# CMU-SAFARI/AirLift

Measured on AMD Instinct MI355X. Metric: reads/sec remapped (150 bp PE), higher is better.
Workload: dtype u8/int32 (int8 SW lanes, u64 hashes)

## Files before the change

### airlift_amd/csrc/al_dev_ksw2.h

```cpp
#pragma once

#define DPP_ROW_BCAST7 0x157

typedef short al_s2 __attribute__((ext_vector_type(2)));
typedef unsigned short al_u2 __attribute__((ext_vector_type(2)));
__device__ __forceinline__ al_s2 pk_s(uint32_t v) { return __builtin_bit_cast(al_s2, v); }
__device__ __forceinline__ uint32_t pk_u(al_s2 v) { return __builtin_bit_cast(uint32_t, v); }
__device__ __forceinline__ uint32_t pk_add(uint32_t a, uint32_t b) { return pk_u(pk_s(a) + pk_s(b)); }
__device__ __forceinline__ uint32_t pk_sub(uint32_t a, uint32_t b) { return pk_u(pk_s(a) - pk_s(b)); }
__device__ __forceinline__ uint32_t pk_max(uint32_t a, uint32_t b) { return pk_u(__builtin_elementwise_max(pk_s(a), pk_s(b))); }
__device__ __forceinline__ uint32_t pk_min(uint32_t a, uint32_t b) { return pk_u(__builtin_elementwise_min(pk_s(a), pk_s(b))); }
__device__ __forceinline__ uint32_t pk_sar8(uint32_t a) { return pk_u(pk_s(a) >> (al_s2)(8)); }
__device__ __forceinline__ uint32_t pk_minu1(uint32_t a) { uint32_t d; asm("v_pk_min_u16 %0, %1, 1 op_sel_hi:[1,0]" : "=v"(d) : "v"(a)); return d; }
__device__ __forceinline__ uint32_t pk_subsat(uint32_t a, uint32_t b) { uint32_t d; asm("v_pk_sub_u16 %0, %1, %2 clamp" : "=v"(d) : "v"(a), "v"(b)); return d; }
__device__ __forceinline__ uint32_t pk_dec(uint32_t a) { uint32_t d; asm("v_pk_sub_u16 %0, %1, 1 op_sel_hi:[1,0]" : "=v"(d) : "v"(a)); return d; }
__device__ __forceinline__ uint32_t pk_mask_eq(uint32_t t, uint32_t v) { return pk_dec(pk_minu1(t ^ v)); }
__device__ __forceinline__ uint32_t pk_mask_in(uint32_t t, uint32_t lo, uint32_t width) { return pk_dec(pk_minu1(pk_subsat(pk_sub(t, lo), width))); }
__device__ __forceinline__ uint32_t d_bfi(uint32_t mask, uint32_t if_set, uint32_t if_clear) { return (if_set & mask) | (if_clear & ~mask); }
__device__ __forceinline__ uint32_t pk_splat(int v) { return (uint32_t)(v & 0xffff) * 0x00010001u; }
__device__ __forceinline__ uint32_t pk_splat8(int v) { return (uint32_t)((v & 0xff) << 8) * 0x00010001u; }
__device__ __forceinline__ unsigned long long d_grp_any(unsigned long long b) { b |= b >> 8; b |= b >> 4; b |= b >> 2; b |= b >> 1; return b & 0x0001000100010001ull; }

template <int NP, class LT, int DIR = 2, bool EXIT = false>
__device__ __forceinline__ void d_ksw_pk(LT &L, const uint8_t *__restrict__ selE, const uint8_t *__restrict__ selO, const int gl, GroupWs &ws, int qlen, int tlen, const AlParams &P,
                                         int w, int zdrop, int end_bonus, int flag, EzD &ez, bool do_bt = true, unsigned long long *xcnt = nullptr)
{
	int q = P.q, e = P.e, q2 = P.q2, e2 = P.e2;
	if (q2 + e2 < q + e) { int t = q; q = q2; q2 = t; t = e; e = e2; e2 = t; }
	const int qe = q + e;
	const int sc_mch = P.a, sc_mis = -P.b;
	if (w < 0) w = tlen > qlen ? tlen : qlen;
	const int tlen_ = (tlen + 15) / 16;
	int n_col_ = qlen < tlen ? qlen : tlen;
	n_col_ = ((n_col_ < w + 1 ? n_col_ : w + 1) + 15) / 16 + 1;
	int long_thres = e != e2 ? (q2 - q) / (e - e2) - 1 : 0;
	if (q2 + e2 + long_thres * e2 > q + e + long_thres * e) ++long_thres;
	const int long_diff = long_thres * (e - e2) - (q2 - q) - e2;
	const bool right = DIR == 2 ? (flag & EZ_RIGHT) != 0 : DIR == 1;
	const uint32_t M1 = pk_splat8(-q - e), M2 = pk_splat8(-q2 - e2), QE = pk_splat8(q + e), QE2 = pk_splat8(q2 + e2), QQ = pk_splat8(q), QQ2 = pk_splat8(q2), MCH = pk_splat8(sc_mch);
	const uint32_t TG0 = right ? 0x00000000u : 0x00070007u, TG1 = right ? 0x00010001u : 0x00060006u, TG2 = right ? 0x00020002u : 0x00050005u,
// ... 235 lines not shown
		const int rows_run = r < n_rows ? r + 1 : n_rows, need = exit_row >= 0 ? exit_row + 1 : rows_run;
		bool differs = false;
		if (exit_row >= 0) {
			const int smax = (int)L.ezc[0], smax_t = (int)L.ezc[1], smax_q = (int)L.ezc[2], smqe = (int)L.ezc[3], smqe_t = (int)L.ezc[4];
			const bool reach_f = !ez.zdropped && ez.mqe + end_bonus > ez.max, reach_s = smqe + end_bonus > smax;
			differs = smax != ez.max || smax_t != ez.max_t || smax_q != ez.max_q || reach_s != reach_f || (reach_f && smqe_t != ez.mqe_t);
		}
		int wn = need, wr = rows_run;
		const bool full = __ballot(1) == ~0ull;
		if (full) { wn = max(wn, __shfl_xor(wn, 16)); wn = max(wn, __shfl_xor(wn, 32)); wr = max(wr, __shfl_xor(wr, 16)); wr = max(wr, __shfl_xor(wr, 32)); }
		if (gl == 0) {
			const int sv = (int)((long long)(n_rows - need) * 100 / n_rows);
			atomicAdd(xcnt + 0, 1ull); if (differs) atomicAdd(xcnt + 1, 1ull);
			atomicAdd(xcnt + 2, (unsigned long long)n_rows); atomicAdd(xcnt + 3, (unsigned long long)need);
			atomicAdd(xcnt + (sv < 25 ? 6 : 7), (sv < 10 || (sv >= 25 && sv < 40)) ? 1ull : 1ull << 32);
		}
		if (full && threadIdx.x == 0) { atomicAdd(xcnt + 4, (unsigned long long)wr); atomicAdd(xcnt + 5, (unsigned long long)wn); }
	}
	GSYNC();
	if (do_bt) {
		const int rev_cigar = !!(flag & EZ_REV_CIGAR);
		CigW cw{L.ezc, 0, AL_LCIG, ws.ezc, 0xffffffffu};
		if (!ez.zdropped && !(flag & EZ_EXTZ_ONLY)) d_backtrack(ptb, n_col_ * 16, qlen, tlen, w, rev_cigar, tlen - 1, qlen - 1, cw);
		else if (!ez.zdropped && (flag & EZ_EXTZ_ONLY) && ez.mqe + end_bonus > ez.max) { ez.reach_end = 1; d_backtrack(ptb, n_col_ * 16, qlen, tlen, w, rev_cigar, ez.mqe_t, qlen - 1, cw); }
		else if (ez.max_t >= 0 && ez.max_q >= 0) d_backtrack(ptb, n_col_ * 16, qlen, tlen, w, rev_cigar, ez.max_t, ez.max_q, cw);
		ez.n_cigar = cw.n; ws.cur_ezc = cw.c;
	}
	GSYNC();
}
```

### airlift_amd/csrc/al_internal.h

```cpp
#pragma once
#include <stdint.h>
#include <stddef.h>
#include <string>
#include <vector>
#include <memory>
#include <utility>
#include <map>
#include <mutex>
#include "../../include/airlift.h"

#define AL_MAX_K 28
static inline int al_sketch_pos_bits(int k) { const int b = 64 - 2 * k; return b > 22 ? 22 : b; }
static inline bool al_sketch_wide(int k, int max_read_len) { const int pb = al_sketch_pos_bits(k); return k > 25 || max_read_len >= (1 << (pb - 1)); }
#define AL_MAX_READ_LEN 32768
#define AL_SEED_TANDEM    (1ULL<<42)
#define AL_SEED_SEG_SHIFT 48
#define AL_SEED_SEG_MASK  (0xffULL<<AL_SEED_SEG_SHIFT)
#define AL_PARENT_UNSET   (-1)
#define AL_PARENT_TMP_PRI (-2)

struct AlSeq { std::string name; uint64_t offset; uint32_t len; };

struct AlDevIndex {
	uint32_t *S4 = nullptr;
// ... 29 lines not shown
	template <class U, class... A> void construct(U *p, A &&...a) { if constexpr (sizeof...(A) == 0) ::new ((void *)p) U; else ::new ((void *)p) U(std::forward<A>(a)...); }
};
typedef std::vector<char, AlNoInit<char>> AlText;
bool al_fasta_load_parallel(const char *fn, int n_threads, std::vector<AlSeq> &seqs, AlText &ascii);
void al_sketch_host(const uint8_t *codes, uint32_t len, int w, int k, uint32_t rid, std::vector<uint64_t> &hash_out, std::vector<uint64_t> &y_out);

struct AlParams {
	int k, w;
	int seed, bw, max_gap, max_gap_ref, max_frag_len, max_chain_skip, max_chain_iter, min_cnt, min_chain_score;
	float mask_level, pri_ratio, max_clip_ratio;
	int best_n, a, b, q, e, q2, e2, sc_ambi, zdrop, zdrop_inv, end_bonus, min_dp_max;
	int pe_ori, pe_bonus, mid_occ, max_occ;
	int dbg;
	int dbg2;
	int dp_exit;
};

struct AlMatch {
	uint32_t off_lo;
	uint32_t n;
	uint32_t q_pos;
	uint32_t flags;
};

struct AlAnchor { uint64_t x, y; };

#define AL_MAX_CIGAR_INLINE 0

struct AlReg {
	int32_t id, cnt, rid, score;
// ... 43 lines not shown
```

### airlift_amd/csrc/al_kernels_align.hip

```cpp
#include <hip/hip_runtime.h>
#include <string.h>
#include <cstring>
#include <rocprim/rocprim.hpp>
#include <stdio.h>
#include <string.h>
#include <math.h>
#include <vector>
#include <type_traits>
#include "al_internal.h"
#include "al_device.h"
#include "al_runtime.h"
#include "al_dev_regs.h"

#define AL_LREG 6
#define AL_LANC 64
#define AL_LCIG 40
#define AL_LPTB 1280
#define AL_GPB 4
#define GW 16
#define KSW_NEG_INF -0x40000000
#define EZ_RIGHT      0x02
#define EZ_EXTZ_ONLY  0x40
#define EZ_REV_CIGAR  0x80
#define GSYNC() __syncthreads()
// ... 1834 lines not shown
					}
				}
				const int wband = (int)(P.bw * 1.5 + 1.);
				const bool runoff = tl >= ql + wband + 1;
				const bool reach = !runoff && sc + P.end_bonus > mx;
				const int ncig = (reach || pos >= 0) ? 1 : 0;
				ExtOut o; o.max = mx; o.max_q = pos; o.max_t = pos; o.mqe_t = ql - 1;
				o.flags_ncig = (uint32_t)(reach ? 1 : 0) | (uint32_t)(runoff ? 2 : 0) | (uint32_t)ncig << 8; o.cig_off = 0;
				o.cig[0] = ncig ? (uint32_t)(reach ? ql : pos + 1) << 4 : 0; o.cig[1] = o.cig[2] = o.cig[3] = o.cig[4] = o.cig[5] = 0;
				E.outs[jb + side] = o;
				return true;
			};
			if (shortcut(0, jl.qlen, jl.tlen)) jl.pad0 = 1;
			if (shortcut(1, jr.qlen, jr.tlen)) jr.pad0 = 1;
		}
		if (r->cnt > 0 && !((P.dbg >> 18) & 1) && (jl.qlen == 0 || jl.pad0) && (jr.qlen == 0 || jr.pad0)) x.job |= 0x80000000u;
		return 0;
	};
	auto commit = [&](const uint32_t s, const int i, const uint32_t jb, const RegExt &x, const ExtJob &jl, const ExtJob &jr) {
		E.rext[B2 + (uint64_t)s * fw.cap + i] = x;
		E.jobs[jb] = jl; E.jobs[jb + 1] = jr;
		const int c0 = (jl.qlen && !jl.pad0) ? d_job_class(jl.qlen, jl.tlen, lane_ok) : AL_NCLS, c1 = (jr.qlen && !jr.pad0) ? d_job_class(jr.qlen, jr.tlen, lane_ok) : AL_NCLS;
		const uint32_t b0 = (uint32_t)std::min(63, (jl.tlen + 15) / 16), b1 = (uint32_t)std::min(63, (jr.tlen + 15) / 16);
		E.job_key[jb] = c0 < AL_NCLS ? ((uint32_t)c0 << 20 | b0 << 14 | 0u << 13 | (uint32_t)std::min(0x1fff, jl.qlen + jl.tlen)) : 0xffffffffu;
		E.job_key[jb + 1] = c1 < AL_NCLS ? ((uint32_t)c1 << 20 | b1 << 14 | 1u << 13 | (uint32_t)std::min(0x1fff, jr.qlen + jr.tlen)) : 0xffffffffu;
		atomicAdd(&s_hist[c0], 1u); atomicAdd(&s_hist[c1], 1u);
		if (c0 == 7 && b0 <= 16) atomicAdd(&s_sub[b0 <= 12 ? 0 : 1], 1u);
		if (c1 == 7 && b1 <= 16) atomicAdd(&s_sub[b1 <= 12 ? 0 : 1], 1u);
		if (c0 < AL_NCLS) atomicAdd(&s_tl[c0], (unsigned)jl.tlen); if (c1 < AL_NCLS) atomicAdd(&s_tl[c1], (unsigned)jr.tlen);
	};
	auto do_seg = [&](const uint32_t s, const AlReg *regs, const AlAnchor *a) {
		const int qlen = (int)rd_len[r0 + s], n = (int)W.reg_cnt[r0 + s];
		const uint32_t *seq = rd_seq + rd_off[r0 + s];
		if (n > 0 && qlen > qmax) { if (!WAVE || lane == 0) atomicAdd(&G.counters[7], 1ULL << 0); slow = true; return; }
		if (!WAVE) {
			for (int i = 0; i < n; ++i) {
				RegExt x; ExtJob jl, jr; const uint32_t jb = jb0 + 2u * n_done;
				const int code = hit(s, i, regs, a, qlen, seq, jb, x, jl, jr);
				if (code) { if (code == 2) atomicAdd(&G.counters[7], 1ULL << 8); slow = true; return; }
				commit(s, i, jb, x, jl, jr); ++n_done;
// ... 151 lines not shown
		} else {
			const ReadAcc Q{seq, rqlen, job.rev, (int)job.qoff};
			for (int t = gl; t < ql + TMAXJ + 16; t += GW) qr[t] = t < ql ? (uint8_t)Q(ql - 1 - t) : 0;
			for (int i = gl; i < tl; i += GW) L.tbuf[i] = (uint8_t)d_seq4(G.S4, job.toff + (uint64_t)i);
		}
		GSYNC();
		EzD ez; d_ez_reset(ez);
		const int flag = job.kind == 0 ? (EZ_EXTZ_ONLY | EZ_RIGHT | EZ_REV_CIGAR) : EZ_EXTZ_ONLY;
		static_assert(TMAXJ == 16 * NB, "the query pad of JobLds is one block row");
		if constexpr (PK) {
			static_assert(NB % 2 == 0, "two blocks per superblock");
			for (int i = gl; i < ql + 2 * TMAXJ + 16; i += GW) { const uint32_t b0 = L.sq[i]; L.selO[i] = (uint8_t)(b0 < 4 ? 4u + b0 : 0x0du); L.sq[i] = (uint8_t)(b0 < 4 ? b0 : 0x0du); }
			GSYNC();
			const unsigned long long w_act = __ballot(1), w_right = __ballot((flag & EZ_RIGHT) != 0);
			unsigned long long *const xcnt = ((P.dbg2 >> 5) & 1) ? G.counters + 24 : nullptr;
			if (w_right == 0) d_ksw_pk<NB / 2, JobLds<QMAXJ, TMAXJ, PK>, 0, (NB >= 12)>(L, L.sq + TMAXJ, L.selO + TMAXJ, gl, ws, ql, tl, P, bw, P.zdrop, P.end_bonus, flag, ez, true, xcnt);
			else if (w_right == w_act) d_ksw_pk<NB / 2, JobLds<QMAXJ, TMAXJ, PK>, 1, (NB >= 12)>(L, L.sq + TMAXJ, L.selO + TMAXJ, gl, ws, ql, tl, P, bw, P.zdrop, P.end_bonus, flag, ez, true, xcnt);
			else d_ksw_pk<NB / 2, JobLds<QMAXJ, TMAXJ, PK>, 2, (NB >= 12)>(L, L.sq + TMAXJ, L.selO + TMAXJ, gl, ws, ql, tl, P, bw, P.zdrop, P.end_bonus, flag, ez, true, xcnt);
		} else
		d_ksw_reg<NB>(L, gl, ws, ql, tl, P, bw, P.zdrop, P.end_bonus, flag, ez);
		ExtOut o;
		o.max = ez.max; o.max_q = ez.max_q; o.max_t = ez.max_t; o.mqe_t = ez.mqe_t;
		o.flags_ncig = (uint32_t)(ez.reach_end ? 1 : 0) | (uint32_t)(ez.zdropped ? 2 : 0) | (uint32_t)ez.n_cigar << 8; o.cig_off = 0;
		for (int i = 0; i < 6; ++i) o.cig[i] = i < ez.n_cigar ? ws.cur_ezc[i] : 0;
		if (ez.n_cigar > 6) {
			unsigned long long off = 0;
			if (gl == 0) off = atomicAdd(G.arena_cnt, (unsigned long long)ez.n_cigar);
			off = __shfl(off, 0, GW);
			if (off + ez.n_cigar <= G.arena_cap) { for (int i = gl; i < ez.n_cigar; i += GW) G.arena[off + i] = ws.cur_ezc[i]; o.cig_off = (uint32_t)off; }
			else { if (gl == 0) atomicAdd(&G.counters[9], 1ULL); o.cig_off = 0xffffffffu; }
		}
		if (gl == 0) E.outs[j] = o;
		GSYNC();
// ... 975 lines not shown
```

### airlift_amd/csrc/al_runtime.h

```cpp
#pragma once
#include <hip/hip_runtime.h>
#include <stdio.h>
#include <vector>
#include <string>
#include <thread>
#include <chrono>
#include "al_internal.h"

inline bool &al_nomem_flag() { static thread_local bool f = false; return f; }

hipError_t al_dev_malloc(void **p, size_t bytes);
#include <atomic>
std::atomic<size_t> *&al_acct();
struct AlAllocSite { const char *file; int line; };
AlAllocSite &al_alloc_site();
struct AlAllocStat { std::atomic<long long> dev_ns{0}, dev_bytes{0}, dev_calls{0}, host_ns{0}, host_bytes{0}, host_calls{0}; };
AlAllocStat &al_alloc_stat();
void al_dev_free(void *p);
double al_long_batch_cap(double reads);
long long al_dev_reserve_room();
hipError_t al_dev_mem_info(size_t *free_b, size_t *total_b);
int al_dev_guard_check();

template <typename T> struct DevBuf {
// ... 156 lines not shown
```

### airlift_amd/csrc/al_runtime.hip

```cpp
#include <hip/hip_runtime.h>
#include <stdio.h>
#include <stdlib.h>
#include <string.h>
#include <sys/stat.h>
#include <cstring>
#include <rocprim/rocprim.hpp>
#include <algorithm>
#include "al_internal.h"
#include "al_device.h"
#include <mutex>
#include <condition_variable>
#include <thread>
#include <atomic>
#include <map>
#include <vector>
#include "al_runtime.h"
#include "al_dev_sort.h"
#include "al_io.h"

extern "C" __global__ void k_sketch(const uint32_t *, const uint64_t *, const uint32_t *, const uint64_t *, AlAnchor *, uint32_t *, int, int, int, int);
extern "C" __global__ void k_seed(const uint64_t *, int, const uint32_t *, const uint32_t *, const uint64_t *, AlAnchor *, const uint32_t *, AlMatch *, uint32_t *, uint32_t *, int32_t *, const uint32_t *, int, int, int, uint32_t *);
#ifndef AL_SPEC_CAP
#define AL_SPEC_CAP 512
#endif
// ... 378 lines not shown
	for (int i = 0; i < 3; ++i) if (hipStreamCreateWithPriority(&c->aux[i], hipStreamNonBlocking, sp) != hipSuccess || hipEventCreateWithFlags(&c->ev_aux[i], hipEventDisableTiming) != hipSuccess) { delete c; return nullptr; }
	for (int i = 0; i < 3; ++i) if (hipStreamCreateWithFlags(&c->ovl[i], hipStreamNonBlocking) != hipSuccess) { delete c; return nullptr; }
	if (hipStreamCreateWithFlags(&c->spec, hipStreamNonBlocking) != hipSuccess || hipStreamCreateWithFlags(&c->spec2, hipStreamNonBlocking) != hipSuccess) { delete c; return nullptr; }
	for (int i = 0; i < 3; ++i) if (hipEventCreateWithFlags(&c->ev_spec[i], hipEventDisableTiming) != hipSuccess) { delete c; return nullptr; }
	for (int i = 0; i < 5; ++i) if (hipEventCreateWithFlags(&c->ev_ovl[i], hipEventDisableTiming) != hipSuccess) { delete c; return nullptr; }
	if (al_upload_index(mi, device, &c->di) != 0) { delete c; return nullptr; }
	AlParams &P = c->P;
	P.k = mi->k; P.w = mi->w; P.seed = opt->seed; P.bw = opt->bw; P.max_gap = opt->max_gap; P.max_gap_ref = opt->max_gap_ref; P.max_frag_len = opt->max_frag_len;
	P.max_chain_skip = opt->max_chain_skip; P.max_chain_iter = opt->max_chain_iter; P.min_cnt = opt->min_cnt; P.min_chain_score = opt->min_chain_score;
	P.mask_level = opt->mask_level; P.pri_ratio = opt->pri_ratio; P.max_clip_ratio = opt->max_clip_ratio; P.best_n = opt->best_n;
	P.a = opt->a; P.b = opt->b; P.q = opt->q; P.e = opt->e; P.q2 = opt->q2; P.e2 = opt->e2; P.sc_ambi = opt->sc_ambi; P.zdrop = opt->zdrop; P.zdrop_inv = opt->zdrop_inv;
	P.end_bonus = opt->end_bonus; P.min_dp_max = opt->min_dp_max; P.pe_ori = opt->pe_ori; P.pe_bonus = opt->pe_bonus; P.mid_occ = opt->mid_occ; P.max_occ = opt->max_occ;
	{ const char *d = getenv("AL_DBG"); P.dbg = d ? atoi(d) : 0; if (P.dbg) fprintf(stderr, "[airlift] AL_DBG=%d: timing experiment, results are NOT valid\n", P.dbg); }
	{ const char *d = getenv("AL_DBG2"); P.dbg2 = d ? atoi(d) : 0; if (P.dbg2 & ~32) fprintf(stderr, "[airlift] AL_DBG2=%d: timing experiment, results are NOT valid\n", P.dbg2); }
	{ const char *d = getenv("AL_DP_EXIT"); P.dp_exit = d ? atoi(d) != 0 : 1; }
	memset(&c->stat, 0, sizeof(c->stat));
	return c;
}

void al_align_state_free(al_ctx_t *c);
static void ctx_release_buffers(al_ctx_t *c)
{
	if (c->stream) (void)hipStreamSynchronize(c->stream);
	if (c->side) (void)hipStreamSynchronize(c->side);
	for (int i = 0; i < 3; ++i) if (c->aux[i]) (void)hipStreamSynchronize(c->aux[i]);
	for (int i = 0; i < 3; ++i) if (c->ovl[i]) (void)hipStreamSynchronize(c->ovl[i]);
	if (c->spec) (void)hipStreamSynchronize(c->spec);
	if (c->spec2) (void)hipStreamSynchronize(c->spec2);
	(void)hipGetLastError();
	al_align_state_free(c);
// ... 90 lines not shown
	al_parallel_for(c->n_threads, (size_t)n_reads, [&](size_t lo, size_t hi, int) {
		for (size_t i = lo; i < hi; ++i) {
			uint32_t *w = c->h_rd_seq.data() + c->h_rd_off[i]; const char *s = seqs[i]; const int L = qlens[i], nw = (L + 7) / 8 + 1;
			for (int b = 0; b < nw; ++b) {
				uint32_t v = 0; const int j0 = b * 8, j1 = j0 + 8 < L ? j0 + 8 : L;
				if (!c->h_flip[i]) for (int j = j0; j < j1; ++j) v |= (uint32_t)nt4[(unsigned char)s[j]] << ((j & 7) << 2);
				else for (int j = j0; j < j1; ++j) { const unsigned cd = nt4[(unsigned char)s[L - 1 - j]]; v |= (uint32_t)(cd < 4 ? 3 - cd : 4) << ((j & 7) << 2); }
				w[b] = v;
			}
		}
	});
	hipStream_t s = c->stream;
	if (c->rd_seq.ensure(words + 1) || c->rd_off.ensure(n_reads + 1) || c->rd_len.ensure(n_reads + 1) || c->frag_first.ensure(n_frag + 1) || c->frag_hash.ensure(n_frag + 1) ||
	    c->mini_off.ensure(n_reads + 1) || c->mini.ensure(mtot + 1) || c->mini_cnt.ensure(n_reads + 1) || c->match.ensure(mtot + 1) || c->heap_ws.ensure(mtot + 1) ||
	    c->frag_nm.ensure(n_frag + 1) || c->frag_na.ensure(n_frag + 1) || c->frag_rep.ensure(n_frag + 1) || c->frag_nu.ensure(n_frag + 1) || c->a_off.ensure(n_frag + 2) ||
	    c->rechain_list.ensure(n_frag + 1) || c->tmp_u32.ensure(n_frag + 2) || c->tmp_u64.ensure(n_frag + 2) || c->counters.ensure(32)) return -1;
	AL_HIP_CHECK(hipMemcpyAsync(c->rd_seq.p, c->h_rd_seq.data(), (words + 1) * 4, hipMemcpyHostToDevice, s));
	AL_HIP_CHECK(hipMemcpyAsync(c->rd_off.p, c->h_rd_off.data(), (n_reads + 1) * 8, hipMemcpyHostToDevice, s));
	AL_HIP_CHECK(hipMemcpyAsync(c->rd_len.p, c->h_rd_len.data(), (n_reads + 1) * 4, hipMemcpyHostToDevice, s));
	AL_HIP_CHECK(hipMemcpyAsync(c->frag_first.p, c->h_frag_first.data(), (n_frag + 1) * 4, hipMemcpyHostToDevice, s));
	AL_HIP_CHECK(hipMemcpyAsync(c->frag_hash.p, c->h_frag_hash.data(), (n_frag + 1) * 4, hipMemcpyHostToDevice, s));
	AL_HIP_CHECK(hipMemcpyAsync(c->mini_off.p, c->h_mini_off.data(), (n_reads + 1) * 8, hipMemcpyHostToDevice, s));
	AL_HIP_CHECK(hipStreamSynchronize(s));
	return 0;
}

struct CastU64 { __host__ __device__ uint64_t operator()(const uint32_t &v) const { return (uint64_t)v; } };

static int scan_u32_to_u64(al_ctx_t *c, const uint32_t *in, uint64_t *out, int n, hipStream_t st = nullptr, DevBuf<unsigned char> *tmp = nullptr)
{
	hipStream_t s_ = st ? st : c->stream; DevBuf<unsigned char> &T_ = tmp ? *tmp : c->scan_tmp;
// ... 622 lines not shown
				TileSched S; for (int k = 0; k < 6; ++k) { S.ent[k] = 0; S.item[k] = 0; } S.ent[6] = n_tie; S.item[6] = n_tie; S.n_items = n_tie;
				if (chain_tiles(c, c->tie_sorted.p, S, nullptr, lmin, false, lds_ok)) return -1;
			} else if (chain_legacy(c, c->tie_sorted.p, (int)n_tie, lds_ok, nullptr)) return -1;
		}
		if (ev(ST_SEG_MERGE)) return -1;
	}
	AL_HIP_CHECK(hipGetLastError());
	return 0;
}
#undef LCH

int al_run_seed_stages(al_ctx_t *c)
{
	hipStream_t s = c->stream;
	AL_HIP_CHECK(hipSetDevice(c->device));
	AL_HIP_CHECK(hipMemsetAsync(c->counters.p, 0, 32 * sizeof(unsigned long long), s));
	AL_HIP_CHECK(hipEventRecord(c->ev[0], s));
	const int nr = c->n_reads, w = c->mi->w, k = c->mi->k;
	const bool sk_wide = al_sketch_wide(k, c->max_rd_len);
	if (nr > 0) hipLaunchKernelGGL(k_sketch, dim3((nr + 63) / 64), dim3(64), (size_t)w * 64 * (sk_wide ? 12 : 8), s, c->rd_seq.p, c->rd_off.p, c->rd_len.p, c->mini_off.p, c->mini.p, c->mini_cnt.p, nr, w, k, sk_wide ? -1 : al_sketch_pos_bits(k));
	AL_HIP_CHECK(hipEventRecord(c->ev[ST_SKETCH + 1], s));
	if (c->n_frag == 0) { for (int i = ST_SEED; i < ST_N; ++i) AL_HIP_CHECK(hipEventRecord(c->ev[i + 1], s)); return 0; }
	if (c->frag_meta.ensure((size_t)c->n_frag + 1)) return -1;
	hipLaunchKernelGGL(k_frag_meta, dim3((c->n_frag + 255) / 256), dim3(256), 0, s, c->frag_first.p, c->rd_len.p, c->n_frag, c->frag_meta.p);
	if (run_seed_chain(c, nullptr, c->n_frag, c->opt.mid_occ, 0, true)) return -1;
	c->n_rechain = 0;
	if (c->opt.max_occ > c->opt.mid_occ) {
		uint32_t *cnt = (uint32_t *)(c->counters.p + 3);
		hipLaunchKernelGGL(k_rechain_test, dim3((c->n_frag + 255) / 256), dim3(256), 0, s, c->chained.p, c->a_off.p, c->u.p, c->uo.p, c->frag_nu.p, c->frag_rep.p, c->frag_first.p, c->n_frag, c->rechain_list.p, cnt);
		uint32_t n = 0;
		AL_HIP_CHECK(hipMemcpyAsync(&n, cnt, 4, hipMemcpyDeviceToHost, s));
// ... 45 lines not shown
	if ((al_tag_kind(c->opt.flag) || (c->opt.flag & AL_F_EQX)) && al_run_tags(c)) return failed();
	for (int i = 0; i < ST_N; ++i) { float ms = 0; if (hipEventElapsedTime(&ms, c->ev[i], c->ev[i + 1]) != hipSuccess) ms = 0; c->ms_stage[i] = ms; }
	float tot = 0; (void)hipEventElapsedTime(&tot, c->ev[0], c->ev[ST_N]); c->ms_total = tot;
	{ float a = 0, b = 0; if (hipEventElapsedTime(&a, c->ev_side[0], c->ev_side[1]) != hipSuccess) a = 0; if (c->n_rechain == 0 || hipEventElapsedTime(&b, c->ev_side[2], c->ev_side[3]) != hipSuccess) b = 0; c->ms_side = a + b; (void)hipGetLastError(); }
	c->ran = true;
	{ static const bool guard = getenv("AL_TEST_GUARD") != nullptr; if (guard && al_dev_guard_check()) fprintf(stderr, "[airlift] GUARD: violations after al_batch_run\n"); }
	unsigned long long h[16]; AL_HIP_CHECK(hipMemcpy(h, c->counters.p, sizeof(h), hipMemcpyDeviceToHost));
	if ((c->P.dbg >> 24) & 1) { unsigned long long t[8]; AL_HIP_CHECK(hipMemcpy(t, c->counters.p + 24, sizeof(t), hipMemcpyDeviceToHost));
		fprintf(stderr, "[airlift] tile kernel profile (cycles of thread 0, all blocks, both passes): setup %llu load %llu cut %llu dp %llu emit %llu copy %llu; tiles %llu\n", t[0], t[1], t[2], t[3], t[4], t[5], t[6]); }
	if ((c->P.dbg2 >> 3) & 1) { unsigned long long t[8]; AL_HIP_CHECK(hipMemcpy(t, c->counters.p + 24, sizeof(t), hipMemcpyDeviceToHost));
		fprintf(stderr, "[airlift] lane chaining kernels (cycles per wavefront, all launches of the batch): setup %llu load %llu recurrence %llu ends/backtrack/order %llu copy %llu; wavefronts %llu\n", t[5] ? t[0] / t[5] : 0, t[5] ? t[1] / t[5] : 0, t[5] ? t[2] / t[5] : 0, t[5] ? t[3] / t[5] : 0, t[5] ? t[4] / t[5] : 0, t[5]); }
	if ((c->P.dbg2 >> 4) & 1) { unsigned long long t[8]; AL_HIP_CHECK(hipMemcpy(t, c->counters.p + 24, sizeof(t), hipMemcpyDeviceToHost));
		fprintf(stderr, "[airlift] k_regs_heavy (lane 0 = mate 0, cycles summed over fragments): gen_regs %llu set_parent %llu squeeze %llu; hits %llu; whole blocks %llu over %llu fragments\n", t[0], t[1], t[2], t[3], t[4], t[5]); }
	if ((c->P.dbg2 >> 5) & 1) { unsigned long long t[8]; AL_HIP_CHECK(hipMemcpy(t, c->counters.p + 24, sizeof(t), hipMemcpyDeviceToHost));
		fprintf(stderr, "[airlift] DP exit shadow (two-cells-per-lane jobs): jobs %llu, differing %llu; rows needed %llu of %llu (%.1f %%); per wavefront %llu of %llu (%.1f %%); jobs saving < 10 %% %llu, 10-25 %% %llu, 25-40 %% %llu, >= 40 %% %llu\n",
		        t[0], t[1], t[3], t[2], t[2] ? 100.0 * (double)t[3] / (double)t[2] : 0.0, t[5], t[4], t[4] ? 100.0 * (double)t[5] / (double)t[4] : 0.0, t[6] & 0xffffffffull, t[6] >> 32, t[7] & 0xffffffffull, t[7] >> 32); }
	if (getenv("AL_TRACE")) { fprintf(stderr, "[airlift] trace: counters"); for (int i = 0; i < 16; ++i) fprintf(stderr, " [%d]=%llu", i, h[i]); fprintf(stderr, " rechain=%u\n", c->n_rechain); }
	al_batch_stat_t &st = c->stat; memset(&st, 0, sizeof(st));
	st.n_frag = c->n_frag; st.n_reads = c->n_reads; st.n_bases = c->n_bases;
	st.n_mini = ~0ULL; st.n_chain = ~0ULL;
	st.n_anchor = c->n_anchor_total; st.n_rechain = c->n_rechain; st.n_heap_fallback = h[0]; st.n_sort_tie_flag = h[1] + h[10];
	st.n_regs_aln = h[4]; st.n_refbases = h[5]; st.n_cigar = h[6];
	st.bytes_in = c->stat_bytes_in; st.bytes_out = 48 * st.n_regs_aln + 4 * st.n_cigar;
	st.ms_total = c->ms_total; st.n_stage = ST_N; st.ms_side_stream = c->ms_side; st.n_chain_fallback = c->n_chain_fallback; c->n_chain_fallback = 0;
	for (int i = 0; i < 10; ++i) { st.dp_jobs[i] = c->stat_dp_jobs[i]; st.dp_target_bases[i] = c->stat_dp_tbases[i]; }
	for (int i = 0; i < ST_N; ++i) st.ms_kernel[i] = c->ms_stage[i];
	return 0;
}

__global__ void k_sum_u32(const uint32_t *a, int n, unsigned long long *out)
{
// ... 203 lines not shown
	c->h_rd_off.resize(n_tok + 1); c->h_mini_off.resize(n_tok + 1); c->h_flip.assign(n_tok, 0);
	c->h_frag_first.resize(n_tok + 1); c->h_frag_hash.resize(n_tok + 1);
	const uint64_t mper = (uint64_t)(read_len >= k ? read_len - k + 1 : 0) + 1;
	for (int i = 0; i <= n_tok; ++i) { c->h_rd_off[i] = (uint64_t)i * wpr; c->h_mini_off[i] = (uint64_t)i * mper; c->h_frag_first[i] = (uint32_t)i; }
	al_parallel_for(c->n_threads, (size_t)n_tok, [&](size_t lo, size_t hi, int) {
		for (size_t i = lo; i < hi; ++i) c->h_frag_hash[i] = qname_hash(qnames ? qnames[i] : nullptr, read_len, c->opt.seed);
	});
	for (int i = 0; i < n_tok; ++i) if (start[i] + (uint64_t)read_len > src->n_bases) { fprintf(stderr, "[airlift] al_batch_upload_windows: window %d leaves the source\n", i); return -2; }
	const uint64_t words = (uint64_t)n_tok * wpr, mtot = (uint64_t)n_tok * mper, bases = (uint64_t)n_tok * read_len;
	c->n_bases = bases; c->mini_total = mtot; c->seq_words = words;
	c->stat_bytes_in = (uint64_t)n_tok * (((uint64_t)read_len * 3 + 7) / 8);
	hipStream_t s = c->stream; const int n_frag = n_tok, n_reads = n_tok;
	if (c->rd_seq.ensure(words + 1) || c->rd_off.ensure(n_reads + 1) || c->rd_len.ensure(n_reads + 1) || c->frag_first.ensure(n_frag + 1) || c->frag_hash.ensure(n_frag + 1) ||
	    c->mini_off.ensure(n_reads + 1) || c->mini.ensure(mtot + 1) || c->mini_cnt.ensure(n_reads + 1) || c->match.ensure(mtot + 1) || c->heap_ws.ensure(mtot + 1) ||
	    c->frag_nm.ensure(n_frag + 1) || c->frag_na.ensure(n_frag + 1) || c->frag_rep.ensure(n_frag + 1) || c->frag_nu.ensure(n_frag + 1) || c->a_off.ensure(n_frag + 2) ||
	    c->rechain_list.ensure(n_frag + 1) || c->tmp_u32.ensure(n_frag + 2) || c->tmp_u64.ensure(n_frag + 2) || c->counters.ensure(32) || c->tmp_u64b.ensure(n_tok + 1)) return -1;
	AL_HIP_CHECK(hipMemcpyAsync(c->tmp_u64b.p, start, (size_t)n_tok * 8, hipMemcpyHostToDevice, s));
	if (words) hipLaunchKernelGGL(k_make_windows, dim3((unsigned)((words + 255) / 256)), dim3(256), 0, s, src->S4, c->tmp_u64b.p, n_tok, read_len, wpr, c->rd_seq.p);
	AL_HIP_CHECK(hipMemsetAsync(c->rd_seq.p + words, 0, 4, s));
	AL_HIP_CHECK(hipMemcpyAsync(c->rd_off.p, c->h_rd_off.data(), (size_t)(n_reads + 1) * 8, hipMemcpyHostToDevice, s));
	AL_HIP_CHECK(hipMemcpyAsync(c->rd_len.p, c->h_rd_len.data(), (size_t)(n_reads + 1) * 4, hipMemcpyHostToDevice, s));
	AL_HIP_CHECK(hipMemcpyAsync(c->frag_first.p, c->h_frag_first.data(), (size_t)(n_frag + 1) * 4, hipMemcpyHostToDevice, s));
	AL_HIP_CHECK(hipMemcpyAsync(c->frag_hash.p, c->h_frag_hash.data(), (size_t)(n_frag + 1) * 4, hipMemcpyHostToDevice, s));
	AL_HIP_CHECK(hipMemcpyAsync(c->mini_off.p, c->h_mini_off.data(), (size_t)(n_reads + 1) * 8, hipMemcpyHostToDevice, s));
	AL_HIP_CHECK(hipStreamSynchronize(s));
	return 0;
}
```

### airlift_amd/csrc/al_stream.hip

```cpp
#include <hip/hip_runtime.h>
#include <stdio.h>
#include <stdlib.h>
#include <string.h>
#include <cstring>
#include <rocprim/rocprim.hpp>
#include <algorithm>
#include <vector>
#include <string>
#include "al_internal.h"
#include "al_device.h"
#include "al_runtime.h"
#include "al_io.h"
#include "al_stream.h"
#include "al_dev_sam.h"

#define NL_TILE 4096

__device__ __forceinline__ uint32_t d_nl_mask(uint32_t x)
{
	const uint32_t y = x ^ 0x0a0a0a0au;
	return ~(((y & 0x7f7f7f7fu) + 0x7f7f7f7fu) | y | 0x7f7f7f7fu);
}
__device__ __forceinline__ uint4 d_load16(const uint8_t *__restrict__ t, uint64_t n, uint64_t at)
{
// ... 404 lines not shown
		AL_HIP_CHECK(hipStreamSynchronize(s));
		res->consumed[i] = e;
	}
	return 0;
}

int al_stream_setup(AlStreamSlot &S, al_ctx_t *c, uint32_t rec_lo, uint32_t rec_hi, uint32_t frag_lo, uint32_t frag_hi)
{
	hipStream_t s = c->stream;
	AL_HIP_CHECK(hipSetDevice(c->device));
	const int n_frag = (int)(frag_hi - frag_lo), n_reads = S.n_files == 2 ? 2 * n_frag : (int)(rec_hi - rec_lo), k = c->mi->k;
	c->n_frag = n_frag; c->n_reads = n_reads; c->ran = false; c->dev_batch = true;
	if (S.rtxt.ensure((size_t)n_reads + 1) || S.rd_info.ensure((size_t)n_reads + 1) || S.rd_frag.ensure((size_t)n_reads + 1) || S.rd_words.ensure((size_t)n_reads + 2) || S.rd_mcnt.ensure((size_t)n_reads + 2)) return -1;
	if (c->rd_off.ensure(n_reads + 2) || c->rd_len.ensure(n_reads + 2) || c->frag_first.ensure(n_frag + 2) || c->frag_hash.ensure(n_frag + 2) || c->mini_off.ensure(n_reads + 2) || c->mini_cnt.ensure(n_reads + 1) ||
	    c->frag_nm.ensure(n_frag + 1) || c->frag_na.ensure(n_frag + 1) || c->frag_rep.ensure(n_frag + 1) || c->frag_nu.ensure(n_frag + 1) || c->a_off.ensure(n_frag + 2) ||
	    c->rechain_list.ensure(n_frag + 1) || c->tmp_u32.ensure(n_frag + 2) || c->tmp_u64.ensure(n_frag + 2) || c->counters.ensure(32)) return -1;
	SetupOut O{S.rtxt.p, S.rd_info.p, S.rd_frag.p, c->rd_len.p, S.rd_words.p, S.rd_mcnt.p, c->frag_first.p, c->frag_hash.p, S.st.p};
	AL_HIP_CHECK(hipMemsetAsync(S.st.p + 4, 0, 4 * 8, s));
	if (S.n_files == 2) hipLaunchKernelGGL(k_setup_pe, dim3((unsigned)((n_frag + 256) / 256)), dim3(256), 0, s, S.txt[0].p, S.frec[0].p + rec_lo, S.frec[1].p + rec_lo, (uint32_t)n_frag, O, k, c->opt.seed, c->opt.pe_ori);
	else hipLaunchKernelGGL(k_setup_se, dim3((unsigned)((n_reads + 256) / 256)), dim3(256), 0, s, S.txt[0].p, S.frec[0].p + rec_lo, S.se_fs.p + rec_lo, S.se_fidx.p + rec_lo, (uint32_t)n_reads, (uint32_t)n_frag, frag_lo, O, k, c->opt.seed, c->opt.pe_ori);
	if (scan_excl_u64(S, S.rd_words.p, c->rd_off.p, (size_t)n_reads + 1, s) || scan_excl_u64(S, S.rd_mcnt.p, c->mini_off.p, (size_t)n_reads + 1, s)) return -1;
	unsigned long long h[4]; uint64_t words = 0, mtot = 0;
	AL_HIP_CHECK(hipMemcpyAsync(h, S.st.p + 4, 32, hipMemcpyDeviceToHost, s));
	AL_HIP_CHECK(hipMemcpyAsync(&words, c->rd_off.p + n_reads, 8, hipMemcpyDeviceToHost, s));
	AL_HIP_CHECK(hipMemcpyAsync(&mtot, c->mini_off.p + n_reads, 8, hipMemcpyDeviceToHost, s));
	AL_HIP_CHECK(hipStreamSynchronize(s));
	c->max_rd_len = (int)h[0]; c->max_qlen_sum = (int)h[1]; c->n_bases = h[2]; c->stat_bytes_in = h[3]; c->seq_words = words; c->mini_total = mtot;
	{
		const int lim = AL_MAX_READ_LEN;
		if (c->max_rd_len >= lim) { fprintf(stderr, "[airlift] a read of %d bases exceeds the limit of the GPU path (%d bases at k = %d)\n", c->max_rd_len, lim - 1, k); return -3; }
	}
// ... 67 lines not shown
```

Measured before the change: 14.97 million.

## Sort DP extension jobs by predicted early-exit hint and enable exit for smaller kernels

Adds a cheap per-job tail-similarity hint, computed by comparing 16 query bases against nearby reference offsets with popcount, and folds it into the sort key for job classes 6 and 7. Jobs with similar expected early-exit behaviour then share a wavefront, so more wavefronts can stop the DP early together. It also enables the early-exit path for the NB>=8 kernels, not only NB>=12, and adds shadow counters per kernel and hint. The cost is extra hint computation and reference reads during job setup, plus a narrower qlen+tlen field in the sort key.

```diff
diff --git a/airlift_amd/csrc/al_dev_ksw2.h b/airlift_amd/csrc/al_dev_ksw2.h
--- a/airlift_amd/csrc/al_dev_ksw2.h
+++ b/airlift_amd/csrc/al_dev_ksw2.h
@@ -23,7 +23,7 @@
 
 template <int NP, class LT, int DIR = 2, bool EXIT = false>
 __device__ __forceinline__ void d_ksw_pk(LT &L, const uint8_t *__restrict__ selE, const uint8_t *__restrict__ selO, const int gl, GroupWs &ws, int qlen, int tlen, const AlParams &P,
-                                         int w, int zdrop, int end_bonus, int flag, EzD &ez, bool do_bt = true, unsigned long long *xcnt = nullptr)
+                                         int w, int zdrop, int end_bonus, int flag, EzD &ez, bool do_bt = true, unsigned long long *xcnt = nullptr, uint32_t xhint = 0)
 {
 	int q = P.q, e = P.e, q2 = P.q2, e2 = P.e2;
 	if (q2 + e2 < q + e) { int t = q; q = q2; q2 = t; t = e; e = e2; e2 = t; }
@@ -289,8 +289,14 @@
 			atomicAdd(xcnt + 0, 1ull); if (differs) atomicAdd(xcnt + 1, 1ull);
 			atomicAdd(xcnt + 2, (unsigned long long)n_rows); atomicAdd(xcnt + 3, (unsigned long long)need);
 			atomicAdd(xcnt + (sv < 25 ? 6 : 7), (sv < 10 || (sv >= 25 && sv < 40)) ? 1ull : 1ull << 32);
-		}
-		if (full && threadIdx.x == 0) { atomicAdd(xcnt + 4, (unsigned long long)wr); atomicAdd(xcnt + 5, (unsigned long long)wn); }
+			const int ob = sv < 10 ? 0 : sv < 25 ? 1 : 2;
+			atomicAdd(xcnt + 16 + 3 * (xhint < 2 ? xhint : 2) + ob, 1ull);
+		}
+		if (full && threadIdx.x == 0) {
+			atomicAdd(xcnt + 4, (unsigned long long)wr); atomicAdd(xcnt + 5, (unsigned long long)wn);
+			constexpr int xk = NP <= 4 ? 0 : NP <= 6 ? 1 : NP <= 8 ? 2 : 3;
+			atomicAdd(xcnt + 8 + 2 * xk, (unsigned long long)wr); atomicAdd(xcnt + 9 + 2 * xk, (unsigned long long)wn);
+		}
 	}
 	GSYNC();
 	if (do_bt) {
diff --git a/airlift_amd/csrc/al_internal.h b/airlift_amd/csrc/al_internal.h
--- a/airlift_amd/csrc/al_internal.h
+++ b/airlift_amd/csrc/al_internal.h
@@ -67,6 +67,7 @@
 	int dbg;
 	int dbg2;
 	int dp_exit;
+	int dp_order;
 };
 
 struct AlMatch {
diff --git a/airlift_amd/csrc/al_kernels_align.hip b/airlift_amd/csrc/al_kernels_align.hip
--- a/airlift_amd/csrc/al_kernels_align.hip
+++ b/airlift_amd/csrc/al_kernels_align.hip
@@ -1872,6 +1872,30 @@
 			if (shortcut(0, jl.qlen, jl.tlen)) jl.pad0 = 1;
 			if (shortcut(1, jr.qlen, jr.tlen)) jr.pad0 = 1;
 		}
+		if (r->cnt > 0 && (P.dp_order || ((P.dbg2 >> 5) & 1))) {
+			const int32_t rid3 = r->rid, rev3 = (r->flags & ALR_REV) ? 1 : 0;
+			const int64_t ref_len3 = (int64_t)G.seq_len[rid3]; const uint64_t ref_off3 = G.seq_off[rid3];
+			const ReadAcc Qt{seq, qlen, rev3, 0};
+			auto tail = [&](const int side, const int ql, const int tl) -> uint8_t {
+				const int wband = (int)(P.bw * 1.5 + 1.);
+				if (tl >= ql + wband + 1) return 2;
+				const int qp = side == 0 ? 0 : qlen - 16;
+				const int64_t tp = side == 0 ? (int64_t)x.rs - x.qs : (int64_t)x.re - x.qe + qlen - 16;
+				if (ql < 16 || tp < 2 || tp + 18 > ref_len3) return 1;
+				const uint32_t q0 = Qt.win8(qp), q1 = Qt.win8(qp + 8);
+				const uint64_t a0 = ref_off3 + (uint64_t)(tp - 2), w0 = a0 >> 3; const int s0 = (int)(a0 & 7);
+				const uint32_t t0 = G.S4[w0], t1 = G.S4[w0 + 1], t2 = G.S4[w0 + 2], t3 = G.S4[w0 + 3];
+				auto tw = [&](const int o) -> uint32_t { const int p = s0 + o, k = p >> 3; const uint32_t lo = k == 0 ? t0 : k == 1 ? t1 : t2, hi = k == 0 ? t1 : k == 1 ? t2 : t3;
+				                                         return (uint32_t)((((uint64_t)hi << 32) | lo) >> ((p & 7) << 2)); };
+				auto mm = [](const uint32_t qw, const uint32_t tw_) -> int { const uint32_t y = (qw ^ tw_) | ((qw | tw_) & 0x44444444u); return __popc((y | y >> 1 | y >> 2) & 0x11111111u); };
+				int best = 16;
+#pragma unroll
+				for (int o = 0; o < 5; ++o) { const int m = mm(q0, tw(o)) + mm(q1, tw(o + 8)); best = m < best ? m : best; }
+				return best <= 1 ? 1 : best <= 4 ? 2 : 0;
+			};
+			if (jl.qlen && !jl.pad0 && jl.tlen > 64) jl.pad1 = tail(0, jl.qlen, jl.tlen);
+			if (jr.qlen && !jr.pad0 && jr.tlen > 64) jr.pad1 = tail(1, jr.qlen, jr.tlen);
+		}
 		if (r->cnt > 0 && !((P.dbg >> 18) & 1) && (jl.qlen == 0 || jl.pad0) && (jr.qlen == 0 || jr.pad0)) x.job |= 0x80000000u;
 		return 0;
 	};
@@ -1880,8 +1904,13 @@
 		E.jobs[jb] = jl; E.jobs[jb + 1] = jr;
 		const int c0 = (jl.qlen && !jl.pad0) ? d_job_class(jl.qlen, jl.tlen, lane_ok) : AL_NCLS, c1 = (jr.qlen && !jr.pad0) ? d_job_class(jr.qlen, jr.tlen, lane_ok) : AL_NCLS;
 		const uint32_t b0 = (uint32_t)std::min(63, (jl.tlen + 15) / 16), b1 = (uint32_t)std::min(63, (jr.tlen + 15) / 16);
-		E.job_key[jb] = c0 < AL_NCLS ? ((uint32_t)c0 << 20 | b0 << 14 | 0u << 13 | (uint32_t)std::min(0x1fff, jl.qlen + jl.tlen)) : 0xffffffffu;
-		E.job_key[jb + 1] = c1 < AL_NCLS ? ((uint32_t)c1 << 20 | b1 << 14 | 1u << 13 | (uint32_t)std::min(0x1fff, jr.qlen + jr.tlen)) : 0xffffffffu;
+		auto key = [&](const int c, const uint32_t b, const uint32_t dir, const ExtJob &j) -> uint32_t {
+			if (c >= AL_NCLS) return 0xffffffffu;
+			if (!P.dp_order || (c != 6 && c != 7)) return (uint32_t)c << 20 | b << 14 | dir << 13 | (uint32_t)std::min(0x1fff, j.qlen + j.tlen);
+			return (uint32_t)c << 20 | b << 14 | (uint32_t)(j.pad1 & 3) << 12 | dir << 11 | (uint32_t)std::min(0x7ff, j.qlen + j.tlen);
+		};
+		E.job_key[jb] = key(c0, b0, 0u, jl);
+		E.job_key[jb + 1] = key(c1, b1, 1u, jr);
 		atomicAdd(&s_hist[c0], 1u); atomicAdd(&s_hist[c1], 1u);
 		if (c0 == 7 && b0 <= 16) atomicAdd(&s_sub[b0 <= 12 ? 0 : 1], 1u);
 		if (c1 == 7 && b1 <= 16) atomicAdd(&s_sub[b1 <= 12 ? 0 : 1], 1u);
@@ -2063,9 +2092,10 @@
 			GSYNC();
 			const unsigned long long w_act = __ballot(1), w_right = __ballot((flag & EZ_RIGHT) != 0);
 			unsigned long long *const xcnt = ((P.dbg2 >> 5) & 1) ? G.counters + 24 : nullptr;
-			if (w_right == 0) d_ksw_pk<NB / 2, JobLds<QMAXJ, TMAXJ, PK>, 0, (NB >= 12)>(L, L.sq + TMAXJ, L.selO + TMAXJ, gl, ws, ql, tl, P, bw, P.zdrop, P.end_bonus, flag, ez, true, xcnt);
-			else if (w_right == w_act) d_ksw_pk<NB / 2, JobLds<QMAXJ, TMAXJ, PK>, 1, (NB >= 12)>(L, L.sq + TMAXJ, L.selO + TMAXJ, gl, ws, ql, tl, P, bw, P.zdrop, P.end_bonus, flag, ez, true, xcnt);
-			else d_ksw_pk<NB / 2, JobLds<QMAXJ, TMAXJ, PK>, 2, (NB >= 12)>(L, L.sq + TMAXJ, L.selO + TMAXJ, gl, ws, ql, tl, P, bw, P.zdrop, P.end_bonus, flag, ez, true, xcnt);
+			const uint32_t xh = job.pad1;
+			if (w_right == 0) d_ksw_pk<NB / 2, JobLds<QMAXJ, TMAXJ, PK>, 0, (NB >= 8)>(L, L.sq + TMAXJ, L.selO + TMAXJ, gl, ws, ql, tl, P, bw, P.zdrop, P.end_bonus, flag, ez, true, xcnt, xh);
+			else if (w_right == w_act) d_ksw_pk<NB / 2, JobLds<QMAXJ, TMAXJ, PK>, 1, (NB >= 8)>(L, L.sq + TMAXJ, L.selO + TMAXJ, gl, ws, ql, tl, P, bw, P.zdrop, P.end_bonus, flag, ez, true, xcnt, xh);
+			else d_ksw_pk<NB / 2, JobLds<QMAXJ, TMAXJ, PK>, 2, (NB >= 8)>(L, L.sq + TMAXJ, L.selO + TMAXJ, gl, ws, ql, tl, P, bw, P.zdrop, P.end_bonus, flag, ez, true, xcnt, xh);
 		} else
 		d_ksw_reg<NB>(L, gl, ws, ql, tl, P, bw, P.zdrop, P.end_bonus, flag, ez);
 		ExtOut o;
diff --git a/airlift_amd/csrc/al_runtime.h b/airlift_amd/csrc/al_runtime.h
--- a/airlift_amd/csrc/al_runtime.h
+++ b/airlift_amd/csrc/al_runtime.h
@@ -6,6 +6,8 @@
 #include <thread>
 #include <chrono>
 #include "al_internal.h"
+
+#define AL_NCOUNTERS 64
 
 inline bool &al_nomem_flag() { static thread_local bool f = false; return f; }
 
diff --git a/airlift_amd/csrc/al_runtime.hip b/airlift_amd/csrc/al_runtime.hip
--- a/airlift_amd/csrc/al_runtime.hip
+++ b/airlift_amd/csrc/al_runtime.hip
@@ -416,6 +416,7 @@
 	{ const char *d = getenv("AL_DBG"); P.dbg = d ? atoi(d) : 0; if (P.dbg) fprintf(stderr, "[airlift] AL_DBG=%d: timing experiment, results are NOT valid\n", P.dbg); }
 	{ const char *d = getenv("AL_DBG2"); P.dbg2 = d ? atoi(d) : 0; if (P.dbg2 & ~32) fprintf(stderr, "[airlift] AL_DBG2=%d: timing experiment, results are NOT valid\n", P.dbg2); }
 	{ const char *d = getenv("AL_DP_EXIT"); P.dp_exit = d ? atoi(d) != 0 : 1; }
+	{ const char *d = getenv("AL_DP_ORDER"); P.dp_order = d ? atoi(d) != 0 : 1; }
 	memset(&c->stat, 0, sizeof(c->stat));
 	return c;
 }
@@ -536,7 +537,7 @@
 	if (c->rd_seq.ensure(words + 1) || c->rd_off.ensure(n_reads + 1) || c->rd_len.ensure(n_reads + 1) || c->frag_first.ensure(n_frag + 1) || c->frag_hash.ensure(n_frag + 1) ||
 	    c->mini_off.ensure(n_reads + 1) || c->mini.ensure(mtot + 1) || c->mini_cnt.ensure(n_reads + 1) || c->match.ensure(mtot + 1) || c->heap_ws.ensure(mtot + 1) ||
 	    c->frag_nm.ensure(n_frag + 1) || c->frag_na.ensure(n_frag + 1) || c->frag_rep.ensure(n_frag + 1) || c->frag_nu.ensure(n_frag + 1) || c->a_off.ensure(n_frag + 2) ||
-	    c->rechain_list.ensure(n_frag + 1) || c->tmp_u32.ensure(n_frag + 2) || c->tmp_u64.ensure(n_frag + 2) || c->counters.ensure(32)) return -1;
+	    c->rechain_list.ensure(n_frag + 1) || c->tmp_u32.ensure(n_frag + 2) || c->tmp_u64.ensure(n_frag + 2) || c->counters.ensure(AL_NCOUNTERS)) return -1;
 	AL_HIP_CHECK(hipMemcpyAsync(c->rd_seq.p, c->h_rd_seq.data(), (words + 1) * 4, hipMemcpyHostToDevice, s));
 	AL_HIP_CHECK(hipMemcpyAsync(c->rd_off.p, c->h_rd_off.data(), (n_reads + 1) * 8, hipMemcpyHostToDevice, s));
 	AL_HIP_CHECK(hipMemcpyAsync(c->rd_len.p, c->h_rd_len.data(), (n_reads + 1) * 4, hipMemcpyHostToDevice, s));
@@ -1189,7 +1190,7 @@
 {
 	hipStream_t s = c->stream;
 	AL_HIP_CHECK(hipSetDevice(c->device));
-	AL_HIP_CHECK(hipMemsetAsync(c->counters.p, 0, 32 * sizeof(unsigned long long), s));
+	AL_HIP_CHECK(hipMemsetAsync(c->counters.p, 0, AL_NCOUNTERS * sizeof(unsigned long long), s));
 	AL_HIP_CHECK(hipEventRecord(c->ev[0], s));
 	const int nr = c->n_reads, w = c->mi->w, k = c->mi->k;
 	const bool sk_wide = al_sketch_wide(k, c->max_rd_len);
@@ -1265,7 +1266,12 @@
 		fprintf(stderr, "[airlift] k_regs_heavy (lane 0 = mate 0, cycles summed over fragments): gen_regs %llu set_parent %llu squeeze %llu; hits %llu; whole blocks %llu over %llu fragments\n", t[0], t[1], t[2], t[3], t[4], t[5]); }
 	if ((c->P.dbg2 >> 5) & 1) { unsigned long long t[8]; AL_HIP_CHECK(hipMemcpy(t, c->counters.p + 24, sizeof(t), hipMemcpyDeviceToHost));
 		fprintf(stderr, "[airlift] DP exit shadow (two-cells-per-lane jobs): jobs %llu, differing %llu; rows needed %llu of %llu (%.1f %%); per wavefront %llu of %llu (%.1f %%); jobs saving < 10 %% %llu, 10-25 %% %llu, 25-40 %% %llu, >= 40 %% %llu\n",
-		        t[0], t[1], t[3], t[2], t[2] ? 100.0 * (double)t[3] / (double)t[2] : 0.0, t[5], t[4], t[4] ? 100.0 * (double)t[5] / (double)t[4] : 0.0, t[6] & 0xffffffffull, t[6] >> 32, t[7] & 0xffffffffull, t[7] >> 32); }
+		        t[0], t[1], t[3], t[2], t[2] ? 100.0 * (double)t[3] / (double)t[2] : 0.0, t[5], t[4], t[4] ? 100.0 * (double)t[5] / (double)t[4] : 0.0, t[6] & 0xffffffffull, t[6] >> 32, t[7] & 0xffffffffull, t[7] >> 32);
+		unsigned long long u[17]; AL_HIP_CHECK(hipMemcpy(u, c->counters.p + 32, sizeof(u), hipMemcpyDeviceToHost));
+		fprintf(stderr, "[airlift] DP exit shadow by kernel and hint (AL_DP_ORDER=%d): wavefront rows needed", c->P.dp_order);
+		static const char *const kn[4] = {"<8>", "<12>", "<16>", "<22>"};
+		for (int k = 0; k < 4; ++k) fprintf(stderr, "%s %s %llu of %llu (%.1f %%)", k ? "," : "", kn[k], u[2 * k + 1], u[2 * k], u[2 * k] ? 100.0 * (double)u[2 * k + 1] / (double)u[2 * k] : 0.0);
+		fprintf(stderr, "; jobs saving < 10 %% / 10-25 %% / >= 25 %%: hint 0 %llu / %llu / %llu, hint 1 %llu / %llu / %llu, hint 2 %llu / %llu / %llu\n", u[8], u[9], u[10], u[11], u[12], u[13], u[14], u[15], u[16]); }
 	if (getenv("AL_TRACE")) { fprintf(stderr, "[airlift] trace: counters"); for (int i = 0; i < 16; ++i) fprintf(stderr, " [%d]=%llu", i, h[i]); fprintf(stderr, " rechain=%u\n", c->n_rechain); }
 	al_batch_stat_t &st = c->stat; memset(&st, 0, sizeof(st));
 	st.n_frag = c->n_frag; st.n_reads = c->n_reads; st.n_bases = c->n_bases;
@@ -1499,7 +1505,7 @@
 	if (c->rd_seq.ensure(words + 1) || c->rd_off.ensure(n_reads + 1) || c->rd_len.ensure(n_reads + 1) || c->frag_first.ensure(n_frag + 1) || c->frag_hash.ensure(n_frag + 1) ||
 	    c->mini_off.ensure(n_reads + 1) || c->mini.ensure(mtot + 1) || c->mini_cnt.ensure(n_reads + 1) || c->match.ensure(mtot + 1) || c->heap_ws.ensure(mtot + 1) ||
 	    c->frag_nm.ensure(n_frag + 1) || c->frag_na.ensure(n_frag + 1) || c->frag_rep.ensure(n_frag + 1) || c->frag_nu.ensure(n_frag + 1) || c->a_off.ensure(n_frag + 2) ||
-	    c->rechain_list.ensure(n_frag + 1) || c->tmp_u32.ensure(n_frag + 2) || c->tmp_u64.ensure(n_frag + 2) || c->counters.ensure(32) || c->tmp_u64b.ensure(n_tok + 1)) return -1;
+	    c->rechain_list.ensure(n_frag + 1) || c->tmp_u32.ensure(n_frag + 2) || c->tmp_u64.ensure(n_frag + 2) || c->counters.ensure(AL_NCOUNTERS) || c->tmp_u64b.ensure(n_tok + 1)) return -1;
 	AL_HIP_CHECK(hipMemcpyAsync(c->tmp_u64b.p, start, (size_t)n_tok * 8, hipMemcpyHostToDevice, s));
 	if (words) hipLaunchKernelGGL(k_make_windows, dim3((unsigned)((words + 255) / 256)), dim3(256), 0, s, src->S4, c->tmp_u64b.p, n_tok, read_len, wpr, c->rd_seq.p);
 	AL_HIP_CHECK(hipMemsetAsync(c->rd_seq.p + words, 0, 4, s));
diff --git a/airlift_amd/csrc/al_stream.hip b/airlift_amd/csrc/al_stream.hip
--- a/airlift_amd/csrc/al_stream.hip
+++ b/airlift_amd/csrc/al_stream.hip
@@ -442,7 +442,7 @@
 	if (S.rtxt.ensure((size_t)n_reads + 1) || S.rd_info.ensure((size_t)n_reads + 1) || S.rd_frag.ensure((size_t)n_reads + 1) || S.rd_words.ensure((size_t)n_reads + 2) || S.rd_mcnt.ensure((size_t)n_reads + 2)) return -1;
 	if (c->rd_off.ensure(n_reads + 2) || c->rd_len.ensure(n_reads + 2) || c->frag_first.ensure(n_frag + 2) || c->frag_hash.ensure(n_frag + 2) || c->mini_off.ensure(n_reads + 2) || c->mini_cnt.ensure(n_reads + 1) ||
 	    c->frag_nm.ensure(n_frag + 1) || c->frag_na.ensure(n_frag + 1) || c->frag_rep.ensure(n_frag + 1) || c->frag_nu.ensure(n_frag + 1) || c->a_off.ensure(n_frag + 2) ||
-	    c->rechain_list.ensure(n_frag + 1) || c->tmp_u32.ensure(n_frag + 2) || c->tmp_u64.ensure(n_frag + 2) || c->counters.ensure(32)) return -1;
+	    c->rechain_list.ensure(n_frag + 1) || c->tmp_u32.ensure(n_frag + 2) || c->tmp_u64.ensure(n_frag + 2) || c->counters.ensure(AL_NCOUNTERS)) return -1;
 	SetupOut O{S.rtxt.p, S.rd_info.p, S.rd_frag.p, c->rd_len.p, S.rd_words.p, S.rd_mcnt.p, c->frag_first.p, c->frag_hash.p, S.st.p};
 	AL_HIP_CHECK(hipMemsetAsync(S.st.p + 4, 0, 4 * 8, s));
 	if (S.n_files == 2) hipLaunchKernelGGL(k_setup_pe, dim3((unsigned)((n_frag + 256) / 256)), dim3(256), 0, s, S.txt[0].p, S.frec[0].p + rec_lo, S.frec[1].p + rec_lo, (uint32_t)n_frag, O, k, c->opt.seed, c->opt.pe_ori);
```

After: 15.11 million (median of 6 runs). About the same (+1.0%).
